# oceanusxiv/pathtracer-rs

Measured on AMD Instinct MI355X. Metric: Mray/s, Cornell Box 1024x1024, 256 spp, depth 15 (Msample/s in config), higher is better.
Workload: dtype f32

## Files before the change

pathtracer-rs_amd/csrc/ptrs_hip.hip:

```cpp
#include <hip/hip_runtime.h>

#include <cstdio>
#include <cstdlib>
#include <cstring>
#include <map>
#include <mutex>
#include <new>
#include <string>
#include <thread>
#include <vector>

#include "pt_render.h"
#include "pt_aov.h"
#include "pt_probe.h"

using namespace pt;

static const unsigned char k_sobol_blob[] = {
#include "sobol_tables_data.inc"
};

namespace {

thread_local std::string g_err;

struct Options {
    int lanes = 0;
    int refill = -1;
    int refill_connect = -1;
    int stack_lds = 8;
    int grid_mult = 0;
    int grid_pct = 0;
    int whole_rounds = 0;
    int persist = 1;
    int node_form = 0;
    int node_order = 0;
    int vote = -1;
    int fused_epilogue = 1;
    int fused_resolve = 1;
    int shade_lds = 1;
    int env_presample = 1;
    int peer_copy = 1;
    int deal = 0;
    int tail = 1;
    int tail_at = -1;
    int tail_paths = 0;
    int workspace_pct = 40;
    int aov_fused_film = 1;
};
Options g_opt;
std::mutex g_opt_mu;
Options options() { std::lock_guard<std::mutex> lk(g_opt_mu); return g_opt; }
struct OptionDesc { const char *name; int Options::*field; int lo, hi; };
const OptionDesc k_options[] = {
    {"lanes", &Options::lanes, 0, 8}, {"refill", &Options::refill, -1, 64}, {"refill_connect", &Options::refill_connect, -1, 64}, {"stack_lds", &Options::stack_lds, 8, 16},
    {"grid_mult", &Options::grid_mult, 0, 64}, {"persist", &Options::persist, 0, 1}, {"whole_rounds", &Options::whole_rounds, 0, 1}, {"grid_pct", &Options::grid_pct, 0, 100}, {"node_form", &Options::node_form, 0, 2}, {"node_order", &Options::node_order, 0, 1}, {"vote", &Options::vote, -1, 2}, {"shade_lds", &Options::shade_lds, 0, 1}, {"fused_epilogue", &Options::fused_epilogue, 0, 1}, {"fused_resolve", &Options::fused_resolve, 0, 1}, {"workspace_pct", &Options::workspace_pct, 1, 90}, {"peer_copy", &Options::peer_copy, 0, 1}, {"env_presample", &Options::env_presample, 0, 1}, {"deal", &Options::deal, 0, 1}, {"tail", &Options::tail, 0, 1}, {"tail_at", &Options::tail_at, -1, 64}, {"tail_paths", &Options::tail_paths, 0, 1 << 20}, {"aov_fused_film", &Options::aov_fused_film, 0, 1},
};

#define HIPCHK(expr)                                                                                             \
    do {                                                                                                          \
        hipError_t e_ = (expr);                                                                                   \
        if (e_ != hipSuccess) {                                                                                   \
            g_err = std::string(#expr) + ": " + hipGetErrorString(e_);                                            \
            return PTRS_ERR_DEVICE;                                                                               \
        }                                                                                                         \
    } while (0)

constexpr int BLOCK = 256, WAVES = BLOCK / 64;

__device__ inline uint32_t rfl(uint32_t v) { return (uint32_t)__builtin_amdgcn_readfirstlane((int)v); }
__device__ inline uint32_t lanes_below(unsigned long long m) { return __builtin_amdgcn_mbcnt_hi((uint32_t)(m >> 32), __builtin_amdgcn_mbcnt_lo((uint32_t)m, 0u)); }
__device__ inline uint32_t wave_push(uint32_t &count, bool pred) {
    const unsigned long long m = __ballot(pred);
    const uint32_t slot = count + lanes_below(m);
    count += (uint32_t)__popcll(m);
    return slot;
}
enum : uint32_t { TK_SUB = 64, TK_SUB_STRIDE = 32, TK_LAUNCH_WORDS = TK_SUB * TK_SUB_STRIDE };
__device__ inline uint32_t seg_next(uint32_t *ticket, uint32_t G) {
    const uint32_t per = (G + TK_SUB - 1u) / TK_SUB;
    const uint32_t home = (blockIdx.x * WAVES + (threadIdx.x >> 6)) & (TK_SUB - 1u);
    for (;;) {
        uint32_t tmp; unsigned long long open;
        asm volatile("v_mbcnt_lo_u32_b32 %0, -1, 0\n\tv_mbcnt_hi_u32_b32 %0, -1, %0\n\tv_lshlrev_b32 %0, 7, %0\n\tglobal_load_dword %0, %0, %2 sc1\n\ts_waitcnt vmcnt(0)\n\tv_cmp_gt_u32 %1, %3, %0"
                     : "=&v"(tmp), "=s"(open) : "s"(ticket), "s"(per) : "memory");
        static_assert(TK_SUB_STRIDE * 4u == 128u, "the asm above shifts the lane id by 7");
        if (open == 0ull) return 0xffffffffu;
        const unsigned long long rot = home ? ((open >> home) | (open << (64u - home))) : open;
        const uint32_t c = (home + (uint32_t)__ffsll((long long)rot) - 1u) & (TK_SUB - 1u);
        uint32_t t = 0;
        if (__lane_id() == 0) t = atomicAdd(ticket + c * TK_SUB_STRIDE, 1u);
        t = rfl(t);
        const uint32_t s = c * per + t;
        if (t < per && s < G) return s;
    }
}
__device__ inline uint32_t *seg_count(const DQueues &Q, uint32_t row, int q, uint32_t G, uint32_t s) { return Q.counts + ((size_t)row * Q_STRIDE + (size_t)q) * G + s; }
enum { TK_EXTEND = 0, TK_CONNECT = 1, TK_SHADE0 = 2, TK_EPILOGUE = 9, TK_RESOLVE = 10, TK_PRESAMPLE = 11, TK_TAIL = 12 };
__device__ inline bool round_is_dead(const DQueues &Q, uint32_t it) { return it > 0u && rfl(Q.alive[it]) == 0u; }

typedef __attribute__((address_space(3))) const v4 lds_v4;
__device__ inline v4 lds_ld(lds_v4 *q) { v4 r; r.x = q->x; r.y = q->y; r.z = q->z; r.w = q->w; return r; }
enum : uint32_t { TOP_LDS_STRIDE = 9 };
struct GeomTop {
    lds_v4 *top; const v4 *nodesv; const DTri *tris; uint32_t ktop;
    __device__ inline void node8(uint32_t i, v4 *o) const {
        if (i < ktop) { lds_v4 *q = top + TOP_LDS_STRIDE * i; for (int k = 0; k < 8; ++k) o[k] = lds_ld(q + k); }
        else { const v4 *q = nodesv + 8u * i; for (int k = 0; k < 8; ++k) o[k] = q[k]; }
    }
    __device__ inline void quad_load(uint32_t i, uint32_t px, uint32_t py, uint32_t pz, v4 &xn, v4 &xf, v4 &yn, v4 &yf, v4 &zn, v4 &zf, v4 &refs, v4 &meta) const {
        if (i < ktop) {
            typedef __attribute__((address_space(3))) const char lds_c;
            lds_c *b = (lds_c *)top + i * (TOP_LDS_STRIDE * 16u);
            xn = lds_ld((lds_v4 *)(b + px)); xf = lds_ld((lds_v4 *)(b + (px ^ 16u)));
            yn = lds_ld((lds_v4 *)(b + py)); yf = lds_ld((lds_v4 *)(b + (py ^ 16u)));
            zn = lds_ld((lds_v4 *)(b + pz)); zf = lds_ld((lds_v4 *)(b + (pz ^ 16u)));
            refs = lds_ld((lds_v4 *)(b + 96u)); meta = lds_ld((lds_v4 *)(b + 112u));
        } else {
            const char *b = reinterpret_cast<const char *>(nodesv);
            const uint32_t off = i * 128u;
            xn = *reinterpret_cast<const v4 *>(b + (size_t)(off + px)); xf = *reinterpret_cast<const v4 *>(b + (size_t)((off + px) ^ 16u));
            yn = *reinterpret_cast<const v4 *>(b + (size_t)(off + py)); yf = *reinterpret_cast<const v4 *>(b + (size_t)((off + py) ^ 16u));
            zn = *reinterpret_cast<const v4 *>(b + (size_t)(off + pz)); zf = *reinterpret_cast<const v4 *>(b + (size_t)((off + pz) ^ 16u));
            refs = *reinterpret_cast<const v4 *>(b + (size_t)(off + 96u)); meta = *reinterpret_cast<const v4 *>(b + (size_t)(off + 112u));
        }
    }
    __device__ inline void node(uint32_t, v4 &, v4 &, v4 &, v4 &) const {}
    __device__ inline void tri(uint32_t k, v4 &a, v4 &b, v4 &c) const { const v4 *q = reinterpret_cast<const v4 *>(tris + k); a = q[0]; b = q[1]; c = q[2]; }
};

struct StackSpill { unsigned long long *p; uint32_t stride; };
template <int D, bool OVF>
struct LdsStack {
    unsigned long long *col, *ovf; uint32_t ovf_stride;
    int n;
    __device__ inline void init(unsigned long long *lds, const StackSpill &sp) { col = lds + threadIdx.x; ovf = OVF ? sp.p + (size_t)blockIdx.x * BLOCK + threadIdx.x : nullptr; ovf_stride = sp.stride; n = 0; }
    __device__ inline void push(uint32_t v, float t) {
        const unsigned long long e = (unsigned long long)v | ((unsigned long long)f2u(t) << 32);
        if (!OVF || n < D) col[n * BLOCK] = e; else ovf[(size_t)(n - D) * ovf_stride] = e;
// ... 591 lines not shown
            __builtin_amdgcn_global_load_lds((gptr *)&pslot(P.pre0, m.e), (lptr *)(lds_pf + (5u * 4u + wv) * 64u), 16, 0, 0);
            __builtin_amdgcn_global_load_lds((gptr *)&pslot(P.pre1, m.e), (lptr *)(lds_pf + (6u * 4u + wv) * 64u), 16, 0, 0);
        }
    };
    const MatEntry *__restrict__ queue = Q.mat[MAT] + (size_t)s * seg_cap;
    const uint32_t n = rfl(*seg_count(Q, it, Q_MAT0 + MAT, Gn, s));
    if (n == 0) return;
    const uint32_t next_base = rfl(*seg_count(Q, it + 1u, Q_EXT, Gn, s)), nee_base = rfl(*seg_count(Q, it, Q_NEE, Gn, s));
    const uint32_t e_next0 = s * seg_cap + next_base, f0 = s * seg_cap + nee_base;
    uint32_t c_next = 0, c_nee = 0, c_shadow = 0, c_mis = 0;
    uint32_t i = lane;
    MatEntry m, m1; m.e = m.pid = m1.e = m1.pid = 0;
    if (i < n) { m = pslot(queue, i); dma(m); }
    if (i + 64u < n) m1 = pslot(queue, i + 64u);
    __builtin_amdgcn_s_waitcnt(0x0F70);
    while (i < n) {
        PathIn in;
        {
            lds_v4 *q = (lds_v4 *)lds_pf + threadIdx.x;
            if (FEAT & FEAT_IMAGE) in.ro = X.ld(q); else in.ro = mkv4(splat3(0.0f), 0.0f);
            in.rd = X.ld(q + BLOCK); in.beta = X.ld(q + 2 * BLOCK);
            const v4 a = X.ld(q + 3 * BLOCK), c = X.ld(q + 4 * BLOCK);
            in.st.x = f2u(a.x); in.st.y = f2u(a.y); in.st.z = f2u(a.z); in.st.w = f2u(a.w);
            in.hit.x = f2u(c.x); in.hit.y = f2u(c.y); in.hit.z = f2u(c.z); in.hit.w = f2u(c.w);
            if ((FEAT & FEAT_INFINITE) && cfg.pre_li != 0xffffffffu) { in.pre0 = X.ld(q + 5 * BLOCK); in.pre1 = X.ld(q + 6 * BLOCK); } else in.pre0 = in.pre1 = mkv4(splat3(0.0f), 0.0f);
        }
        __builtin_amdgcn_s_waitcnt(0xC07F);
        const uint32_t i2 = i + 64u;
        if (i2 < n) dma(m1);
        MatEntry m2; m2.e = m2.pid = 0;
        if (i2 + 64u < n) m2 = pslot(queue, i2 + 64u);
#ifdef PTRS_STAMPS
        const ShadeResult r = shade_item<MAT, FEAT>(R, S, C, sc, P, m.pid, in, X, stamp_acc, stamp_last);
#else
        const ShadeResult r = shade_item<MAT, FEAT>(R, S, C, sc, P, m.pid, in, X);
#endif
        err_dim = err_dim || r.err_dim;
        const uint32_t e_next = e_next0 + wave_push(c_next, r.next), f = f0 + wave_push(c_nee, r.nee);
        X.before_stores();
        store_shade_out(P, par ^ 1u, r, e_next, f);
        if (r.next) pslot(Q.ext[par ^ 1u], e_next) = m.pid;
        if (r.nee) pslot(Q.nee, f) = r.nee_entry(m.pid);
#ifdef PTRS_STAMPS
        { const unsigned long long t_ = __builtin_amdgcn_s_memtime(); stamp_acc[8] += t_ - stamp_last; stamp_last = t_; stamp_acc[10] += 1; }
#endif
        c_shadow += (uint32_t)__popcll(__ballot(r.shadow));
        c_mis += (uint32_t)__popcll(__ballot(r.mis));
        if (R.row_cost && (r.shadow || r.mis)) atomicAdd(R.row_cost + sample_row_of(R, m.pid), (r.shadow ? 1u : 0u) + (r.mis ? 1u : 0u));
        i = i2; m = m1; m1 = m2;
    }
    if (lane == 0) {
        *seg_count(Q, it + 1u, Q_EXT, Gn, s) = next_base + c_next;
        if (c_next) Q.alive[it + 1u] = 1u;
        *seg_count(Q, it, Q_NEE, Gn, s) = nee_base + c_nee;
        *seg_count(Q, it, Q_SHADOW, Gn, s) += c_shadow;
        *seg_count(Q, it, Q_MIS, Gn, s) += c_mis;
    }
}

template <int MAT, int FEAT, bool ENVPRE>
__global__ __launch_bounds__(BLOCK, (ShadeWaves<MAT, FEAT>::N)) void k_shade(DParams R, DSampler S, DCamera C, DScene sc, DPaths P, DQueues Q, uint32_t it, uint32_t seg_cap, ShadeLdsCfg cfg, uint32_t Gn, uint32_t *ticket) {
    __shared__ v4 lds_pf[ShadeLdsSizes<FEAT, ENVPRE>::NPF * BLOCK];
    __shared__ uint32_t lds_sob[SH_SOB_WORDS];
    __shared__ v4 lds_tri[SH_TRI_V4];
    __shared__ v4 lds_light[SH_LIGHTS * SH_LIGHT_V4];
    __shared__ float lds_marg[ShadeLdsSizes<FEAT, ENVPRE>::MARG ? SH_MARG_WORDS : 1];
    bool err_dim = false;
    if (round_is_dead(Q, it)) return;
    const ShadeCtxLds<ENVPRE> X = stage_shade_tables<FEAT, ENVPRE>(S, sc, cfg, lds_sob, lds_tri, lds_light, lds_marg);
    __syncthreads();
#ifdef PTRS_STAMPS
    unsigned long long stamp_acc[12] = {0, 0, 0, 0, 0, 0, 0, 0, 0, 0, 0, 0}, stamp_last = __builtin_amdgcn_s_memtime();
    for (uint32_t s = seg_next(ticket, Gn); s < Gn; s = seg_next(ticket, Gn)) shade_segment<MAT, FEAT, ENVPRE>(R, S, C, sc, P, Q, it, seg_cap, Gn, s, X, lds_pf, err_dim, stamp_acc, stamp_last);
#else
    for (uint32_t s = seg_next(ticket, Gn); s < Gn; s = seg_next(ticket, Gn)) shade_segment<MAT, FEAT, ENVPRE>(R, S, C, sc, P, Q, it, seg_cap, Gn, s, X, lds_pf, err_dim);
#endif
    if (err_dim) atomicOr(&Q.stats[CNT_ERR], (unsigned long long)PTRS_ERRFLAG_SOBOL_DIM);
#ifdef PTRS_STAMPS
    { const unsigned long long t_ = __builtin_amdgcn_s_memtime(); stamp_acc[11] += t_ - stamp_last; }
    if ((threadIdx.x & 63u) == 0) for (int k = 0; k < 12; ++k) atomicAdd(&Q.stats[CNT_STAMP0 + k], stamp_acc[k]);
#endif
}

template <int MAT, int FEAT, int GEOM, bool OVF, int DEPTH = 8>
__global__ __launch_bounds__(BLOCK, 2) void k_tail(DParams R, DSampler S, DCamera C, DScene sc, StackSpill spill, DPaths P, DQueues Q, uint32_t it0, uint32_t it_end, uint32_t seg_cap, uint32_t thresh_e, uint32_t thresh_c,
                                                   uint32_t kinds_mask, ShadeLdsCfg cfg, uint32_t Gn, uint32_t *ticket) {
    constexpr int FEAT_T = FEAT_SIMPLE;
    constexpr bool VOTE_C = GEOM == 0;
    __shared__ unsigned long long lds_stack[DEPTH * BLOCK];
    __shared__ v4 lds_geom[TravLds<DEPTH, GEOM>::V4];
    __shared__ v4 lds_pf[ShadeLdsSizes<FEAT, false>::NPF * BLOCK];
    __shared__ uint32_t lds_sob[4];
    __shared__ v4 lds_tri[SH_TRI_V4];
    __shared__ v4 lds_light[SH_LIGHTS * SH_LIGHT_V4];
    __shared__ float lds_marg[ShadeLdsSizes<FEAT, false>::MARG ? SH_MARG_WORDS : 1];
    if (round_is_dead(Q, it0)) return;
    LdsGeom LG; LG.root = LG.tri0 = LG.tri_copy = 0;
    const GeomTop GG = stage_top(sc, lds_geom, TravLds<DEPTH, GEOM>::TOP);
    if (GEOM > 0) LG = stage_lds_form(sc, lds_geom);
    cfg.sob_n = 0;
    const ShadeCtxLds<false> X = stage_shade_tables<FEAT, false>(S, sc, cfg, lds_sob, lds_tri, lds_light, lds_marg);
    __syncthreads();
    LdsStack<DEPTH, OVF> stk; stk.init(lds_stack, spill);
    uint32_t nn = 0, nt = 0; StepCount stepc;
    bool err_dim = false;
#ifdef PTRS_STAMPS
    unsigned long long stamp_acc[12] = {0, 0, 0, 0, 0, 0, 0, 0, 0, 0, 0, 0}, stamp_last = __builtin_amdgcn_s_memtime();
#endif
    for (uint32_t s = seg_next(ticket, Gn); s < Gn; s = seg_next(ticket, Gn)) {
        for (uint32_t it = it0; it < it_end; ++it) {
            if (rfl(*(volatile uint32_t *)seg_count(Q, it, Q_EXT, Gn, s)) == 0u) break;
#ifdef PTRS_STAMPS_EXT
            { unsigned long long xs[12] = {0, 0, 0, 0, 0, 0, 0, 0, 0, 0, 0, 0}, xs_last = 0; extend_segment<FEAT_T, DEPTH, OVF, GEOM, true>(R, sc, P, Q, it, seg_cap, thresh_e, kinds_mask, Gn, s, GG, LG, stk, nn, nt, stepc PT_XS_ARGS); }
#else
            extend_segment<FEAT_T, DEPTH, OVF, GEOM, true>(R, sc, P, Q, it, seg_cap, thresh_e, kinds_mask, Gn, s, GG, LG, stk, nn, nt, stepc);
#endif
            __threadfence_block();
#ifdef PTRS_STAMPS
            shade_segment<MAT, FEAT, false>(R, S, C, sc, P, Q, it, seg_cap, Gn, s, X, lds_pf, err_dim, stamp_acc, stamp_last);
#else
            shade_segment<MAT, FEAT, false>(R, S, C, sc, P, Q, it, seg_cap, Gn, s, X, lds_pf, err_dim);
#endif
            __threadfence_block();
            connect_segment<FEAT_T, DEPTH, OVF, GEOM, VOTE_C>(sc, P, Q, it, seg_cap, thresh_c, 1u, Gn, s, GG, LG, stk, nn, nt, stepc);
            __threadfence_block();
        }
    }
    if (err_dim) atomicOr(&Q.stats[CNT_ERR], (unsigned long long)PTRS_ERRFLAG_SOBOL_DIM);
    if (R.counters_on) { atomicAdd(&Q.stats[CNT_NODES], (unsigned long long)nn); atomicAdd(&Q.stats[CNT_TRIS], (unsigned long long)nt); atomicAdd(&Q.stats[CNT_NODE_STEPS], (unsigned long long)stepc.node_steps); atomicAdd(&Q.stats[CNT_NODE_VISITS], (unsigned long long)stepc.node_visits); atomicAdd(&Q.stats[CNT_TRI_STEPS], (unsigned long long)stepc.tri_steps); }
}

template <int FEAT>
__global__ __launch_bounds__(BLOCK) void k_env_presample(DSampler S, DScene sc, DPaths P, DQueues Q, uint32_t it, uint32_t seg_cap, uint32_t nee_kinds, uint32_t env_li, ShadeLdsCfg cfg, uint32_t Gn, uint32_t *ticket) {
    __shared__ float lds_marg[SH_MARG_WORDS];
    __shared__ uint32_t lds_sob[SH_SOB_WORDS];
    if (round_is_dead(Q, it)) return;
    const DLight &Le = sc.lights[env_li];
    {
        const uint32_t stride = sob_stride(cfg.sob_nib), nw = cfg.sob_nib * 16u;
        for (uint32_t i = threadIdx.x; i < cfg.sob_n * stride; i += BLOCK) { const uint32_t d = i / stride, w = i - d * stride; lds_sob[i] = w < nw ? S.nibtab[((size_t)(cfg.sob_lo + d) * SOBOL_NIBBLES) * 16u + w] : 0u; }
        const uint32_t nv = (uint32_t)Le.nv, gv = Le.guide_v;
        for (uint32_t i = threadIdx.x; i < nv; i += BLOCK) lds_marg[i] = sc.distdata[Le.fint_off + i];
        for (uint32_t i = threadIdx.x; i < nv + 1u; i += BLOCK) lds_marg[SH_MARG_N + i] = sc.distdata[Le.mcdf_off + i];
        for (uint32_t i = threadIdx.x; i < gv + 1u; i += BLOCK) lds_marg[2u * SH_MARG_N + 1u + i] = sc.distdata[Le.mguide_off + i];
    }
    __syncthreads();
    InfMarginal marg; marg.func = lds_marg; marg.cdf = lds_marg + SH_MARG_N; marg.guide = lds_marg + 2 * SH_MARG_N + 1;
    ShadeCtxLds<false> X; X.sob = (lds_u32 *)lds_sob; X.tris = nullptr; X.lights = nullptr; X.cfg = cfg; X.marg = marg;
    const uint32_t lane = __lane_id();
    for (uint32_t s = seg_next(ticket, Gn); s < Gn; s = seg_next(ticket, Gn)) {
        for (int m = 0; m < 6; ++m) {
            if (!(nee_kinds & (1u << m))) continue;
            const MatEntry *__restrict__ queue = Q.mat[m] + (size_t)s * seg_cap;
            const uint32_t n = rfl(*seg_count(Q, it, Q_MAT0 + m, Gn, s));
            for (uint32_t i = lane; i < n; i += 64u) {
                const MatEntry me = pslot(queue, i);
                const u4 stv = pslot(P.st, me.pid);
                const uint32_t field = f2u(pslot(P.ray_d[it & 1u], me.e).w) & ST_DIM_MASK;
                const VertexDims V = vertex_dims(field, true);
                const uint64_t index = (uint64_t)stv.x | ((uint64_t)stv.y << 32);
                const uint32_t dc[1] = {V.nee[4]};
                float uc[1];
                X.sobol<1>(S, index, dc, stv.w, uc);
                const float fl = floor_(uc[0] * (float)sc.n_lights);
                uint32_t li = fl > 0.0f ? (uint32_t)fl : 0u;
                if (li > sc.n_lights - 1u) li = sc.n_lights - 1u;
                if (li != env_li) continue;
                const uint32_t dn[2] = {V.nee[0], V.nee[1]};
                float u[2];
                X.sobol<2>(S, index, dn, stv.w, u);
                f3 wi, rgb; float pdf;
                const bool ok = inf_light_sample(sc, Le, mk2(u[0], u[1]), wi, pdf, rgb, &marg);
                pslot(P.pre0, me.e) = mkv4(wi, pdf);
                pslot(P.pre1, me.e) = mkv4(rgb, u2f(ok ? 1u : 0u));
            }
        }
    }
}

__global__ __launch_bounds__(BLOCK) void k_reduce_counts(const uint32_t *__restrict__ counts, uint32_t G, uint32_t *__restrict__ totals) {
    __shared__ uint32_t acc;
    if (threadIdx.x == 0) acc = 0;
    __syncthreads();
    uint32_t v = 0;
    for (uint32_t b = threadIdx.x; b < G; b += BLOCK) v += counts[(size_t)blockIdx.x * G + b];
    for (int off = 32; off > 0; off >>= 1) v += (uint32_t)__shfl_down((int)v, off);
    if ((threadIdx.x & 63) == 0) atomicAdd(&acc, v);
    __syncthreads();
    if (threadIdx.x == 0) totals[blockIdx.x] = acc;
}

__global__ __launch_bounds__(BLOCK) void k_film(DParams R, DSampler S, DPaths P, const float *__restrict__ table, v4 *film, int32_t y0, int32_t y1, int32_t tiles_x) {
// ... 546 lines not shown
        (void)hipMemsetAsync(Q.tickets, 0, ((size_t)rows * Q_STRIDE * TK_LAUNCH_WORDS + rows) * 4, stream);
    }
    void generate() { t0(T_AUX); hipLaunchKernelGGL(k_generate, dim3((G + WAVES - 1) / WAVES), dim3(BLOCK), 0, stream, R, S, C, P, Q, seg_cap, G, (uint32_t)deal_by_region()); t1(); }
    int deal_by_region() const { return opt.deal; }

    typedef void (*TravFn)(DParams, DScene, StackSpill, DPaths, DQueues, uint32_t, uint32_t, uint32_t, uint32_t, uint32_t, uint32_t *);
#define PTRS_PICK(K, D, O, GE) (v ? (TravFn)K<FEAT, D, O, GE, true> : (TravFn)K<FEAT, D, O, GE, false>)
#define PTRS_PICK_ALL(K) (ps->stack_lds == 9 ? PTRS_PICK(K, 9, false, 544) : ps->stack_lds == 8 ? (geom4 <= 640 ? (ovf ? PTRS_PICK(K, 8, true, 640) : PTRS_PICK(K, 8, false, 640)) : geom4 <= 1536 ? (ovf ? PTRS_PICK(K, 8, true, 1536) : PTRS_PICK(K, 8, false, 1536)) : (ovf ? PTRS_PICK(K, 8, true, 0) : PTRS_PICK(K, 8, false, 0))) \
                                              : (ovf ? PTRS_PICK(K, 16, true, 0) : PTRS_PICK(K, 16, false, 0)))
    template <int FEAT> TravFn pick_extend(bool v, bool ovf) { return PTRS_PICK_ALL(k_extend_rf); }
    template <int FEAT> TravFn pick_connect(bool v, bool ovf) { return PTRS_PICK_ALL(k_connect_rf); }
#undef PTRS_PICK_ALL
#undef PTRS_PICK
    StackSpill lane_spill() { StackSpill sp = ps->spill; if (sp.p) sp.p += (size_t)cur * ps->spill_lane_elems; return sp; }

    template <int FEAT> void extend_t(uint32_t it) {
        const StackSpill sp = lane_spill();
        const uint32_t epi_mask = opt.fused_epilogue ? kinds_mask : 0u;
        const TravFn fn = pick_extend<FEAT>(vote, sp.p != nullptr);
        hipLaunchKernelGGL(fn, dim3(persistent_grid(fn, T_EXTEND)), dim3(BLOCK), 0, stream, R, sc, sp, P, Q, it, seg_cap, refill, epi_mask, G, ticket(it, TK_EXTEND));
        if (epi_mask) return;
        t1(); t0(T_AUX);
        hipLaunchKernelGGL((k_epilogue<FEAT>), dim3(persistent_grid(k_epilogue<FEAT>, T_AUX)), dim3(BLOCK), 0, stream, R, sc, P, Q, it, kinds_mask, seg_cap, G, ticket(it, TK_EPILOGUE));
    }
    void extend(uint32_t it) { t0(T_EXTEND); if (feat_trace == FEAT_FULL) extend_t<FEAT_FULL>(it); else if (feat_trace == FEAT_IMG_ENV) extend_t<FEAT_IMG_ENV>(it); else extend_t<FEAT_SIMPLE>(it); t1(); }
    template <int FEAT> void connect_t(uint32_t it) {
        const StackSpill sp = lane_spill();
        const uint32_t fused = (opt.fused_epilogue && opt.fused_resolve) ? 1u : 0u;
        const TravFn fn = pick_connect<FEAT>(vote_connect, sp.p != nullptr);
        hipLaunchKernelGGL(fn, dim3(persistent_grid(fn, T_CONNECT)), dim3(BLOCK), 0, stream, R, sc, sp, P, Q, it, seg_cap, refill_connect, fused, G, ticket(it, TK_CONNECT));
        if (fused) return;
        t1(); t0(T_AUX);
        hipLaunchKernelGGL((k_resolve<FEAT>), dim3(persistent_grid(k_resolve<FEAT>, T_AUX)), dim3(BLOCK), 0, stream, sc, P, Q, it, seg_cap, G, ticket(it, TK_RESOLVE));
    }
    void connect(uint32_t it) { t0(T_CONNECT); if (feat_trace == FEAT_FULL) connect_t<FEAT_FULL>(it); else if (feat_trace == FEAT_IMG_ENV) connect_t<FEAT_IMG_ENV>(it); else connect_t<FEAT_SIMPLE>(it); t1(); }
    ShadeLdsCfg shade_cfg(uint32_t it) const {
        ShadeLdsCfg c;
        c.sob_nib = (2u * S.log2_res + (31u - (uint32_t)__builtin_clz(S.spp)) <= 32u) ? 8u : (uint32_t)SOBOL_NIBBLES;
        const uint32_t cap = SH_SOB_WORDS / sob_stride(c.sob_nib), top = std::min<uint32_t>(1024u, 3u + 8u * it + 9u);
        c.sob_lo = top > cap ? top - cap : 0u; c.sob_n = top - c.sob_lo;
        c.tri_lds = (sc.n_prims * SH_TRI_REC_V4 <= SH_TRI_V4 && opt.shade_lds) ? 1u : 0u;
        c.n_lights_lds = opt.shade_lds ? std::min<uint32_t>(sc.n_lights, SH_LIGHTS) : 0u;
        if (!opt.shade_lds) c.sob_n = 0;
        c.pre_li = presample_li();
        c.marg_li = 0xffffffffu;
        if (opt.shade_lds && !ps->H.inf_lights.empty()) {
            const DLight &Le = ps->H.lights[ps->H.inf_lights[0]];
            if (Le.nv >= 1 && (uint32_t)Le.nv <= SH_MARG_N && Le.guide_v >= 1 && Le.guide_v <= SH_MARG_N) c.marg_li = ps->H.inf_lights[0];
        }
        return c;
    }
    typedef void (*ShadeFn)(DParams, DSampler, DCamera, DScene, DPaths, DQueues, uint32_t, uint32_t, ShadeLdsCfg, uint32_t, uint32_t *);
    template <int FEAT, bool ENVPRE> ShadeFn shade_fn_t(int kind) {
        switch (kind) {
            case 0: return k_shade<0, FEAT, ENVPRE>;
            case 1: return k_shade<1, FEAT, ENVPRE>;
            case 2: return k_shade<2, FEAT, ENVPRE>;
            case 3: return k_shade<3, FEAT, ENVPRE>;
            case 4: return k_shade<4, FEAT, ENVPRE>;
            default: return k_shade<5, FEAT, ENVPRE>;
        }
    }
    bool env_presampled_only() const { return presample_li() != 0xffffffffu && ps->H.inf_lights.size() == 1; }
    ShadeFn shade_fn(int kind) {
        if (feat == FEAT_SIMPLE) return shade_fn_t<FEAT_SIMPLE, false>(kind);
        if (feat == FEAT_IMG) return shade_fn_t<FEAT_IMG, false>(kind);
        if (feat == FEAT_IMG_ENV) return env_presampled_only() ? shade_fn_t<FEAT_IMG_ENV, true>(kind) : shade_fn_t<FEAT_IMG_ENV, false>(kind);
        return env_presampled_only() ? shade_fn_t<FEAT_FULL, true>(kind) : shade_fn_t<FEAT_FULL, false>(kind);
    }
    uint32_t presample_li() const {
        if (!opt.env_presample || !(feat & FEAT_INFINITE) || S.kind != PTRS_SAMPLER_SOBOL || ps->H.inf_lights.empty()) return 0xffffffffu;
        const DLight &Le = ps->H.lights[ps->H.inf_lights[0]];
        return (Le.nv >= 1 && (uint32_t)Le.nv <= SH_MARG_N && Le.guide_v >= 1 && Le.guide_v <= SH_MARG_N) ? ps->H.inf_lights[0] : 0xffffffffu;
    }
    void presample(uint32_t it) {
        const uint32_t li = presample_li();
        const uint32_t nee_kinds = kinds_mask & 0x3fu & ~((1u << PTRS_MAT_MIRROR) | (1u << PTRS_MAT_GLASS));
        if (li == 0xffffffffu || !nee_kinds) return;
        t0(T_AUX);
        if (feat == FEAT_IMG_ENV) hipLaunchKernelGGL((k_env_presample<FEAT_IMG_ENV>), dim3(persistent_grid(k_env_presample<FEAT_IMG_ENV>, T_AUX)), dim3(BLOCK), 0, stream, S, sc, P, Q, it, seg_cap, nee_kinds, li, shade_cfg(it), G, ticket(it, TK_PRESAMPLE));
        else hipLaunchKernelGGL((k_env_presample<FEAT_FULL>), dim3(persistent_grid(k_env_presample<FEAT_FULL>, T_AUX)), dim3(BLOCK), 0, stream, S, sc, P, Q, it, seg_cap, nee_kinds, li, shade_cfg(it), G, ticket(it, TK_PRESAMPLE));
        t1();
    }
    typedef void (*TailFn)(DParams, DSampler, DCamera, DScene, StackSpill, DPaths, DQueues, uint32_t, uint32_t, uint32_t, uint32_t, uint32_t, uint32_t, ShadeLdsCfg, uint32_t, uint32_t *);
    enum : uint32_t { TAIL_PATHS_DEFAULT = 192 };
    TailFn tail_fn() {
        if (!opt.tail || !opt.fused_epilogue || !opt.fused_resolve || !opt.shade_lds || !opt.persist || (ps->stack_lds != 8 && ps->stack_lds != 9) || feat_trace != FEAT_SIMPLE || S.kind != PTRS_SAMPLER_SOBOL) return nullptr;
        int kind = -1;
        for (int k = 0; k < 7; ++k) if (ps->H.kinds_present[k]) { if (kind >= 0) return nullptr; kind = k; }
        const bool ovf = ps->spill.p != nullptr;
        if (ps->stack_lds == 9) return (kind == PTRS_MAT_MATTE && feat == FEAT_SIMPLE) ? (TailFn)k_tail<PTRS_MAT_MATTE, FEAT_SIMPLE, 544, false, 9> : nullptr;
        if (kind == PTRS_MAT_MATTE && feat == FEAT_SIMPLE) {
            if (geom4 <= 640) return ovf ? (TailFn)k_tail<PTRS_MAT_MATTE, FEAT_SIMPLE, 640, true> : (TailFn)k_tail<PTRS_MAT_MATTE, FEAT_SIMPLE, 640, false>;
            if (geom4 <= 1536) return ovf ? (TailFn)k_tail<PTRS_MAT_MATTE, FEAT_SIMPLE, 1536, true> : (TailFn)k_tail<PTRS_MAT_MATTE, FEAT_SIMPLE, 1536, false>;
            return ovf ? (TailFn)k_tail<PTRS_MAT_MATTE, FEAT_SIMPLE, 0, true> : (TailFn)k_tail<PTRS_MAT_MATTE, FEAT_SIMPLE, 0, false>;
        }
        if (kind == PTRS_MAT_DISNEY && feat == FEAT_IMG && geom4 > 1536) return ovf ? (TailFn)k_tail<PTRS_MAT_DISNEY, FEAT_IMG, 0, true> : (TailFn)k_tail<PTRS_MAT_DISNEY, FEAT_IMG, 0, false>;
        return nullptr;
    }
    uint32_t tail_round(uint32_t n_paths, uint32_t n_rounds) {
        if (!tail_fn()) return 0xffffffffu;
        if (opt.tail_at >= 0) return (uint32_t)opt.tail_at < n_rounds ? (uint32_t)opt.tail_at : 0xffffffffu;
        const double limit = (double)(opt.tail_paths > 0 ? (uint32_t)opt.tail_paths : (uint32_t)TAIL_PATHS_DEFAULT) * (double)G;
        const std::vector<double> &f = ps->alive_frac;
        for (uint32_t it = 0; it < n_rounds && it < f.size(); ++it) if (f[it] * (double)n_paths <= limit) return it;
        return 0xffffffffu;
    }
    uint32_t tail_at_last = 0xffffffffu;
    void tail(uint32_t it0, uint32_t it_end) {
        const TailFn fn = tail_fn();
        if (!fn) return;
        t0(T_TAIL);
        hipLaunchKernelGGL(fn, dim3(persistent_grid(fn, T_TAIL)), dim3(BLOCK), 0, stream, R, S, C, sc, lane_spill(), P, Q, it0, it_end, seg_cap, refill, refill_connect, kinds_mask & 0x3fu, shade_cfg(it0), G, ticket(it0, TK_TAIL));
        t1();
        tail_at_last = it0;
    }
    void learn(const uint32_t *counts, uint32_t n_rows, uint32_t n_paths) {
        if (!n_paths || n_paths < 4096u) return;
        std::vector<double> f(n_rows);
        for (uint32_t i = 0; i < n_rows; ++i) f[i] = (double)counts[(size_t)i * Q_STRIDE + Q_EXT] / (double)n_paths;
        ps->alive_frac.swap(f);
    }
    void shade(uint32_t it, int kind) {
        t0(T_SHADE);
        if (kind > 5) kind = 5;
        const ShadeFn fn = shade_fn(kind);
        hipLaunchKernelGGL(fn, dim3(persistent_grid(fn, T_SHADE)), dim3(BLOCK), 0, stream, R, S, C, sc, P, Q, it, seg_cap, shade_cfg(it), G, ticket(it, TK_SHADE0 + kind));
        t1();
    }
    void reduce_counts(uint32_t n_rows) { hipLaunchKernelGGL(k_reduce_counts, dim3(n_rows * Q_STRIDE), dim3(BLOCK), 0, stream, (const uint32_t *)Q.counts, G, (uint32_t *)ps->totals[cur].p); }
    uint32_t read_count(uint32_t it, int q) {
        std::vector<uint32_t> seg(G);
        (void)hipMemcpyAsync(seg.data(), Q.counts + ((size_t)it * Q_STRIDE + (size_t)q) * G, (size_t)G * 4, hipMemcpyDeviceToHost, stream);
        if (hipStreamSynchronize(stream) != hipSuccess) { rc = PTRS_ERR_DEVICE; return 0; }
        uint64_t t = 0; for (uint32_t v : seg) t += v;
        return t > 0xffffffffull ? 0xffffffffu : (uint32_t)t;
    }
    void read_counts(uint32_t *dst, uint32_t n_rows) {
        reduce_counts(n_rows);
        (void)hipMemcpyAsync(dst, ps->totals[cur].p, (size_t)n_rows * Q_STRIDE * 4, hipMemcpyDeviceToHost, stream);
        if (hipStreamSynchronize(stream) != hipSuccess) rc = PTRS_ERR_DEVICE;
    }
    void film(v4 *film_px, int32_t y0, int32_t y1) {
        const int32_t tiles_x = (R.W + 15) / 16, tiles_y = (y1 - y0 + 15) / 16;
        if (n_lanes > 1 && film_prev) (void)hipStreamWaitEvent(stream, film_prev, 0);
        t0(T_FILM); hipLaunchKernelGGL(k_film, dim3((uint32_t)tiles_x * (uint32_t)tiles_y), dim3(BLOCK), 0, stream, R, S, P, (const float *)ps->table.p, film_px, y0, y1, tiles_x); t1();
        if (n_lanes > 1) { film_prev = ps->lane_ev[cur]; (void)hipEventRecord(film_prev, stream); }
    }
    PtrsFilmPixel *host_film = nullptr; int32_t film_w = 0;
    void publish_rows(v4 *film_px, int32_t y0, int32_t y1) {
        if (!host_film || hipStreamSynchronize(stream) != hipSuccess) { rc = host_film ? PTRS_ERR_DEVICE : rc; return; }
        const size_t off = (size_t)y0 * (size_t)film_w, cnt = (size_t)(y1 - y0) * (size_t)film_w;
        if (hipMemcpyAsync(host_film + off, film_px + off, cnt * sizeof(PtrsFilmPixel), hipMemcpyDeviceToHost, stream) != hipSuccess || hipStreamSynchronize(stream) != hipSuccess) rc = PTRS_ERR_DEVICE;
    }
    void dump_rays(uint32_t it, const RayDump &d) {
        DevBuf cnt;
        if (cnt.ensure(16) != PTRS_OK) { rc = PTRS_ERR_DEVICE; return; }
        (void)hipMemsetAsync(cnt.p, 0, 16, stream);
        hipLaunchKernelGGL(k_dump_rays, dim3((G + WAVES - 1) / WAVES), dim3(BLOCK), 0, stream, P, Q, it, seg_cap, G, d.max_rays, d.out, (uint32_t *)cnt.p);
        uint32_t n = 0;
        if (hipMemcpyAsync(&n, cnt.p, 4, hipMemcpyDeviceToHost, stream) != hipSuccess || hipStreamSynchronize(stream) != hipSuccess) rc = PTRS_ERR_DEVICE;
        *d.n_out = n < d.max_rays ? n : d.max_rays;
        cnt.release();
    }
    bool aov_band = false;
    int aov_band_begin(uint64_t n, std::string &err) {
        for (auto &b : ps->aov_band) if ((rc = b.ensure((size_t)n * 16)) != PTRS_OK) { err = g_err + " (feature-plane band arrays)"; return rc; }
        if ((rc = ps->aov_band_pfilm.ensure((size_t)n * 8)) != PTRS_OK) { err = g_err + " (feature-plane band arrays)"; return rc; }
        aov_band = true;
        return PTRS_OK;
    }
    DAov aov_arrays(bool depth_plane) const {
        DAov A;
        if (aov_band) { A.albedo = (v4 *)ps->aov_band[0].p; A.normal = (v4 *)ps->aov_band[1].p; A.pos = (v4 *)ps->aov_band[2].p; A.depthp = depth_plane ? (v4 *)ps->aov_band[3].p : nullptr; A.pfilm = (f2a *)ps->aov_band_pfilm.p; }
        else { A.albedo = P.sh_o; A.normal = P.sh_d; A.pos = P.mis_o; A.depthp = depth_plane ? P.mis_d : nullptr; A.pfilm = nullptr; }
        return A;
    }
    bool aov_depth_plane(uint32_t planes) const { return !opt.aov_fused_film && (planes & PTRS_AOV_DEPTH) != 0; }
    void aov(uint32_t planes, uint32_t off) {
        t0(T_AUX);
        const DAov A = aov_arrays(aov_depth_plane(planes));
        if (feat == FEAT_SIMPLE) hipLaunchKernelGGL((k_aov<FEAT_SIMPLE>), dim3((G + WAVES - 1) / WAVES), dim3(BLOCK), 0, stream, R, C, sc, P, Q, A, off, seg_cap, G);
        else hipLaunchKernelGGL((k_aov<FEAT_FULL>), dim3((G + WAVES - 1) / WAVES), dim3(BLOCK), 0, stream, R, C, sc, P, Q, A, off, seg_cap, G);
        t1();
    }
    void film_aov(uint32_t planes, const DAovFilm &films, int32_t y0, int32_t y1, const DParams &Rf ) {
        const int32_t tiles_x = (R.W + 15) / 16, tiles_y = (y1 - y0 + 15) / 16;
        const DAov A = aov_arrays(aov_depth_plane(planes));
        DPaths Pf = P;
        if (A.pfilm) Pf.pfilm = A.pfilm;
        if (n_lanes > 1 && film_prev) (void)hipStreamWaitEvent(stream, film_prev, 0);
        if (opt.aov_fused_film) {
            DAovFilm F = films;
            for (uint32_t k = 0; k < AOV_PLANES; ++k) if (!(planes & (1u << k))) F.plane[k] = nullptr;
            t0(T_FILM); hipLaunchKernelGGL(k_film_aov, dim3((uint32_t)tiles_x * (uint32_t)tiles_y), dim3(BLOCK), 0, stream, Rf, S, Pf, A, (const float *)ps->table.p, F, y0, y1, tiles_x); t1();
        } else {
// ... 44 lines not shown
int do_render(PtrsScene *ps, const PtrsCamera *cam, const PtrsRenderParams *prm, v4 *film_dev, float *samples_dev, hipStream_t stream, PtrsStats *stats, const int32_t *single_pixel = nullptr,
              const RenderProgress *progress = nullptr, PtrsFilmPixel *host_film = nullptr, int share = 1, const RayDump *dump = nullptr, uint32_t *row_cost_dev = nullptr) {
    if (!ps || !cam || !prm || (!film_dev && !single_pixel && !row_cost_dev)) { g_err = "null argument"; return PTRS_ERR_INVALID; }
    HIPCHK(hipSetDevice(ps->device));
    HipBackend be;
    be.ps = ps; be.stream = stream; be.opt = scene_options(ps); be.host_film = host_film; be.film_w = prm->width; be.share = share;
    if (dump && be.opt.lanes == 0) be.opt.lanes = 1;
    int rc = get_sobol(ps->device, &be.sob);
    if (rc != PTRS_OK) return rc;
    std::string err;
    rc = render_impl(be, ps->sc, ps->H, ps->H.max_depth, *cam, *prm, film_dev, samples_dev, stats, err, progress, dump, single_pixel, row_cost_dev);
    if (rc != PTRS_OK) { if (!err.empty()) g_err = err; return rc; }
    if (be.rc != PTRS_OK) { if (g_err.empty()) g_err = "device error during render"; return be.rc; }
    return PTRS_OK;
}

int aov_check_args(PtrsScene *scene, const PtrsCamera *camera, const PtrsRenderParams *params, uint32_t planes, const void *const *plane_ptrs) {
    if (!scene || !camera || !params) { g_err = "null argument"; return PTRS_ERR_INVALID; }
    if (planes == 0u || (planes & ~(uint32_t)(PTRS_AOV_ALBEDO | PTRS_AOV_NORMAL | PTRS_AOV_DEPTH)) != 0u) { g_err = "planes must be a non-empty set of PTRS_AOV_* bits"; return PTRS_ERR_INVALID; }
    for (uint32_t k = 0; k < AOV_PLANES; ++k)
        if ((planes & (1u << k)) && (!plane_ptrs || !plane_ptrs[k])) { g_err = "null plane pointer for a requested plane"; return PTRS_ERR_INVALID; }
    int ndev = 0;
    if (hipGetDeviceCount(&ndev) != hipSuccess || ndev <= 0) { g_err = "no HIP device available (this library has no CPU fallback)"; return PTRS_ERR_DEVICE; }
    return PTRS_OK;
}

int do_render_aov(PtrsScene *ps, const PtrsCamera *cam, const PtrsRenderParams *prm, uint32_t planes, const DAovFilm &films, float *samples_dev, hipStream_t stream, PtrsStats *stats) {
    HIPCHK(hipSetDevice(ps->device));
    HipBackend be;
    be.ps = ps; be.stream = stream; be.opt = scene_options(ps); be.film_w = prm->width;
    int rc = get_sobol(ps->device, &be.sob);
    if (rc != PTRS_OK) return rc;
    std::string err;
    rc = render_aov_impl(be, ps->sc, ps->H, ps->H.max_depth, *cam, *prm, planes, films, samples_dev, stats, err);
    if (rc != PTRS_OK) { if (!err.empty()) g_err = err; return rc; }
    if (be.rc != PTRS_OK) { if (g_err.empty()) g_err = "device error during render"; return be.rc; }
    return PTRS_OK;
}

template <class F> int guarded(F &&f) {
    try { return f(); }
    catch (const std::bad_alloc &) { g_err = "out of host memory"; return PTRS_ERR_DEVICE; }
    catch (const std::exception &e) { g_err = std::string("internal error: ") + e.what(); return PTRS_ERR_INVALID; }
    catch (...) { g_err = "internal error"; return PTRS_ERR_INVALID; }
}

}

extern "C" {

int ptrs_abi_version(void) { return PTRS_ABI_VERSION; }
#ifndef PTRS_BUILD_ID
#define PTRS_BUILD_ID "unknown"
#endif
const char *ptrs_build_id(void) { return PTRS_BUILD_ID; }
const char *ptrs_last_error(void) { return g_err.c_str(); }

int ptrs_abi_sizeof(int which) {
    switch (which) {
        case 0: return (int)sizeof(PtrsTexture); case 1: return (int)sizeof(PtrsMaterial); case 2: return (int)sizeof(PtrsMesh);
        case 3: return (int)sizeof(PtrsLight); case 4: return (int)sizeof(PtrsBvhNode); case 5: return (int)sizeof(PtrsSceneDesc);
        case 6: return (int)sizeof(PtrsCamera); case 7: return (int)sizeof(PtrsRenderParams); case 8: return (int)sizeof(PtrsStats);
        case 9: return (int)sizeof(PtrsHit); case 10: return (int)sizeof(PtrsFilmPixel);
        default: return -1;
    }
}

int ptrs_set_option(const char *name, int64_t value) {
    if (!name) { g_err = "null option name"; return PTRS_ERR_INVALID; }
    for (const OptionDesc &o : k_options)
        if (!std::strcmp(name, o.name)) {
            if (value < o.lo || value > o.hi) { g_err = std::string("option ") + name + ": value outside [" + std::to_string(o.lo) + ", " + std::to_string(o.hi) + "]"; return PTRS_ERR_INVALID; }
            std::lock_guard<std::mutex> lk(g_opt_mu);
            g_opt.*(o.field) = (int)value;
            return PTRS_OK;
        }
    g_err = std::string("unknown option ") + name;
    return PTRS_ERR_INVALID;
}

int ptrs_get_option(const char *name, int64_t *value) {
    if (!name || !value) { g_err = "null argument"; return PTRS_ERR_INVALID; }
    for (const OptionDesc &o : k_options)
        if (!std::strcmp(name, o.name)) { std::lock_guard<std::mutex> lk(g_opt_mu); *value = g_opt.*(o.field); return PTRS_OK; }
    g_err = std::string("unknown option ") + name;
    return PTRS_ERR_INVALID;
}

static int scene_create_impl(const PtrsSceneDesc *desc, int32_t device, PtrsScene **out);
int ptrs_scene_create(const PtrsSceneDesc *desc, int32_t device, PtrsScene **out) { return guarded([&]() { return scene_create_impl(desc, device, out); }); }
static int scene_create_impl(const PtrsSceneDesc *desc, int32_t device, PtrsScene **out) {
    if (!desc || !out) { g_err = "null argument"; return PTRS_ERR_INVALID; }
    int ndev = 0;
    if (hipGetDeviceCount(&ndev) != hipSuccess || ndev <= 0) { g_err = "no HIP device available (this library has no CPU fallback)"; return PTRS_ERR_DEVICE; }
    if (device < 0 || device >= ndev) { g_err = "device ordinal out of range"; return PTRS_ERR_INVALID; }
    HIPCHK(hipSetDevice(device));
    PtrsScene *ps = new PtrsScene();
    ps->device = device;
    const Options opt = options();
    int rc = build_host_scene(*desc, ps->H, g_err, opt.node_form, opt.node_order);
    if (rc != PTRS_OK) { delete ps; return rc; }
    hipDeviceProp_t prop;
    if (hipGetDeviceProperties(&prop, device) == hipSuccess && prop.multiProcessorCount > 0) ps->n_cu = prop.multiProcessorCount;
    HostScene &H = ps->H;
    if ((rc = upload(ps->nodes2, H.nodes2)) || (rc = upload(ps->nodes4, H.nodes4)) || (rc = upload(ps->nodes, H.nodes)) || (rc = upload(ps->tris, H.tris)) || (rc = upload(ps->shade, H.shade)) || (rc = upload(ps->mats, H.mats)) ||
        (rc = upload(ps->texs, H.texs)) || (rc = upload(ps->levels, H.levels)) || (rc = upload(ps->texdata, H.texdata)) || (rc = upload(ps->lights, H.lights)) ||
        (rc = upload(ps->distdata, H.distdata)) || (rc = upload(ps->inf, H.inf_lights))) { delete ps; return rc; }
    DScene &sc = ps->sc;
    sc.nodes2 = (const DNode2 *)ps->nodes2.p; sc.n_nodes2 = (uint32_t)H.nodes2.size(); sc.nodes4 = (const DNode4 *)ps->nodes4.p; sc.n_nodes4 = (uint32_t)H.nodes4.size();
    sc.nodes = (const DNode *)ps->nodes.p; sc.tris = (const DTri *)ps->tris.p; sc.shade = (const DTriShade *)ps->shade.p; sc.mats = (const DMaterial *)ps->mats.p;
    sc.texs = (const DTexture *)ps->texs.p; sc.levels = (const DTexLevel *)ps->levels.p; sc.texdata = (const float *)ps->texdata.p; sc.lights = (const DLight *)ps->lights.p;
    sc.distdata = (const float *)ps->distdata.p; sc.inf_lights = (const uint32_t *)ps->inf.p;
    sc.n_nodes = (uint32_t)H.nodes.size(); sc.n_prims = (uint32_t)H.tris.size(); sc.n_lights = (uint32_t)H.lights.size(); sc.n_inf = (uint32_t)H.inf_lights.size();
    ps->stack_lds = (H.use_quad && opt.stack_lds == 16) ? 16u : 8u;
    if (!H.use_quad && opt.stack_lds != 16 && H.stack_bound == 9u && LN_V4 * (uint32_t)H.nodes2.size() + 9u * (uint32_t)H.tris.size() <= 544u) ps->stack_lds = 9u;
    if (H.stack_bound > ps->stack_lds) {
        const size_t threads = (size_t)ps->n_cu * 8 * BLOCK;
        ps->spill_lane_elems = threads * (size_t)(H.stack_bound - ps->stack_lds);
        if ((rc = ps->stack_spill.ensure(ps->spill_lane_elems * sizeof(unsigned long long))) != PTRS_OK) { delete ps; return rc; }
        ps->spill.p = (unsigned long long *)ps->stack_spill.p; ps->spill.stride = (uint32_t)threads;
    }
    *out = ps;
    return PTRS_OK;
}

void ptrs_scene_destroy(PtrsScene *scene) {
    if (!scene) return;
    (void)hipSetDevice(scene->device);
    delete scene;
}

int ptrs_scene_info(PtrsScene *scene, uint64_t *n_nodes, uint64_t *max_depth, uint64_t *n_tris) {
    if (!scene) { g_err = "null scene"; return PTRS_ERR_INVALID; }
    if (n_nodes) *n_nodes = scene->H.nodes.size();
    if (max_depth) *max_depth = scene->H.max_depth;
    if (n_tris) *n_tris = scene->H.tris.size();
    return PTRS_OK;
}

int ptrs_render_device(PtrsScene *scene, const PtrsCamera *camera, const PtrsRenderParams *params, void *film_inout_device, void *hip_stream, PtrsStats *stats) {
    return guarded([&]() { return do_render(scene, camera, params, (v4 *)film_inout_device, nullptr, (hipStream_t)hip_stream, stats); });
}

static int render_samples_impl(PtrsScene *scene, const PtrsCamera *camera, const PtrsRenderParams *params, PtrsFilmPixel *film_inout, float *sample_rgb, PtrsStats *stats);
int ptrs_render_samples(PtrsScene *scene, const PtrsCamera *camera, const PtrsRenderParams *params, PtrsFilmPixel *film_inout, float *sample_rgb, PtrsStats *stats) {
    return guarded([&]() { return render_samples_impl(scene, camera, params, film_inout, sample_rgb, stats); });
}
static int render_samples_impl(PtrsScene *scene, const PtrsCamera *camera, const PtrsRenderParams *params, PtrsFilmPixel *film_inout, float *sample_rgb, PtrsStats *stats) {
    if (!scene || !params || !film_inout) { g_err = "null argument"; return PTRS_ERR_INVALID; }
    HIPCHK(hipSetDevice(scene->device));
    const size_t npx = (size_t)params->width * (size_t)params->height;
    int rc = scene->film_tmp.ensure(npx * sizeof(PtrsFilmPixel));
    if (rc != PTRS_OK) return rc;
    int32_t rb = params->row_begin, re = params->row_end;
    if (re <= rb) { rb = 0; re = params->height; }
    if (rb < 0 || re > params->height) { g_err = "row band outside the film"; return PTRS_ERR_INVALID; }
    const size_t band_off = (size_t)rb * (size_t)params->width, band_px = (size_t)(re - rb) * (size_t)params->width;
    HIPCHK(hipMemcpy((PtrsFilmPixel *)scene->film_tmp.p + band_off, film_inout + band_off, band_px * sizeof(PtrsFilmPixel), hipMemcpyHostToDevice));
    float *sdev = nullptr; size_t sbytes = 0;
    if (sample_rgb) {
        const SampleGrid g = make_sample_grid(params->width, params->height, params->spp);
        const size_t spp = params->sampler == PTRS_SAMPLER_STRATIFIED ? (size_t)std::max(params->spp, 1) : (size_t)g.spp;
        sbytes = (size_t)g.NX * (size_t)g.NY * spp * 3 * sizeof(float);
        if ((rc = scene->samples_tmp.ensure(sbytes)) != PTRS_OK) return rc;
        HIPCHK(hipMemset(scene->samples_tmp.p, 0, sbytes));
        sdev = (float *)scene->samples_tmp.p;
    }
// ... 522 lines not shown
```

Before: 12570.

## Add grouped tail segments with wave-level queue merging and sized tail grid

After: 12580, median of 6. No clear change (+0.1%).

```diff
diff --git a/pathtracer-rs_amd/csrc/pt_tail_group.h b/pathtracer-rs_amd/csrc/pt_tail_group.h
--- /dev/null
+++ b/pathtracer-rs_amd/csrc/pt_tail_group.h
@@ -0,0 +1,33 @@
+#pragma once
+#include <stdint.h>
+
+#include "../../include/ptrs_detmath.h"
+
+namespace pt {
+
+enum : uint32_t { TAIL_GROUP_MAX = 64 };
+
+PT_HD uint32_t tail_group_tickets(uint32_t G, uint32_t k) { return (G + k - 1u) / k; }
+
+struct TailGroup { uint32_t s0, s1; };
+PT_HD TailGroup tail_group_of(uint32_t g, uint32_t k, uint32_t G) {
+    TailGroup t; t.s0 = g * k; t.s1 = t.s0 + k < G ? t.s0 + k : G;
+    return t;
+}
+
+PT_HD uint32_t tail_group_push(uint32_t off, uint32_t n, uint32_t seg_cap) {
+    if (off == 0xffffffffu || n > seg_cap || off + n > seg_cap) return 0xffffffffu;
+    return off + n;
+}
+PT_HD bool tail_group_merges(uint32_t total) { return total != 0xffffffffu; }
+
+PT_HD uint32_t tail_group_src(uint32_t s, uint32_t seg_cap, uint32_t i) { return s * seg_cap + i; }
+PT_HD uint32_t tail_group_dst(const TailGroup &t, uint32_t seg_cap, uint32_t off, uint32_t i) { return t.s0 * seg_cap + off + i; }
+
+PT_HD uint32_t tail_group_plan(const TailGroup &t, const uint32_t *counts, uint32_t seg_cap, uint32_t *off) {
+    uint32_t run = 0;
+    for (uint32_t j = 0; j < t.s1 - t.s0; ++j) { off[j] = run; run = tail_group_push(run, counts[j], seg_cap); }
+    return run;
+}
+
+}
diff --git a/pathtracer-rs_amd/csrc/ptrs_hip.hip b/pathtracer-rs_amd/csrc/ptrs_hip.hip
--- a/pathtracer-rs_amd/csrc/ptrs_hip.hip
+++ b/pathtracer-rs_amd/csrc/ptrs_hip.hip
@@ -13,6 +13,7 @@
 #include "pt_render.h"
 #include "pt_aov.h"
 #include "pt_probe.h"
+#include "pt_tail_group.h"
 
 using namespace pt;
 
@@ -45,16 +46,18 @@
     int tail = 1;
     int tail_at = -1;
     int tail_paths = 0;
+    int tail_group = 0;
     int workspace_pct = 40;
     int aov_fused_film = 1;
 };
+enum : int { TAIL_GROUP_DEFAULT = 1 };
 Options g_opt;
 std::mutex g_opt_mu;
 Options options() { std::lock_guard<std::mutex> lk(g_opt_mu); return g_opt; }
 struct OptionDesc { const char *name; int Options::*field; int lo, hi; };
 const OptionDesc k_options[] = {
     {"lanes", &Options::lanes, 0, 8}, {"refill", &Options::refill, -1, 64}, {"refill_connect", &Options::refill_connect, -1, 64}, {"stack_lds", &Options::stack_lds, 8, 16},
-    {"grid_mult", &Options::grid_mult, 0, 64}, {"persist", &Options::persist, 0, 1}, {"whole_rounds", &Options::whole_rounds, 0, 1}, {"grid_pct", &Options::grid_pct, 0, 100}, {"node_form", &Options::node_form, 0, 2}, {"node_order", &Options::node_order, 0, 1}, {"vote", &Options::vote, -1, 2}, {"shade_lds", &Options::shade_lds, 0, 1}, {"fused_epilogue", &Options::fused_epilogue, 0, 1}, {"fused_resolve", &Options::fused_resolve, 0, 1}, {"workspace_pct", &Options::workspace_pct, 1, 90}, {"peer_copy", &Options::peer_copy, 0, 1}, {"env_presample", &Options::env_presample, 0, 1}, {"deal", &Options::deal, 0, 1}, {"tail", &Options::tail, 0, 1}, {"tail_at", &Options::tail_at, -1, 64}, {"tail_paths", &Options::tail_paths, 0, 1 << 20}, {"aov_fused_film", &Options::aov_fused_film, 0, 1},
+    {"grid_mult", &Options::grid_mult, 0, 64}, {"persist", &Options::persist, 0, 1}, {"whole_rounds", &Options::whole_rounds, 0, 1}, {"grid_pct", &Options::grid_pct, 0, 100}, {"node_form", &Options::node_form, 0, 2}, {"node_order", &Options::node_order, 0, 1}, {"vote", &Options::vote, -1, 2}, {"shade_lds", &Options::shade_lds, 0, 1}, {"fused_epilogue", &Options::fused_epilogue, 0, 1}, {"fused_resolve", &Options::fused_resolve, 0, 1}, {"workspace_pct", &Options::workspace_pct, 1, 90}, {"peer_copy", &Options::peer_copy, 0, 1}, {"env_presample", &Options::env_presample, 0, 1}, {"deal", &Options::deal, 0, 1}, {"tail", &Options::tail, 0, 1}, {"tail_at", &Options::tail_at, -1, 64}, {"tail_paths", &Options::tail_paths, 0, 1 << 20}, {"tail_group", &Options::tail_group, 0, (int)TAIL_GROUP_MAX}, {"aov_fused_film", &Options::aov_fused_film, 0, 1},
 };
 
 #define HIPCHK(expr)                                                                                             \
@@ -812,9 +815,37 @@
 #endif
 }
 
+__device__ inline bool tail_merge_wave(const DPaths &P, const DQueues &Q, uint32_t it0, uint32_t seg_cap, uint32_t Gn, const TailGroup &tg) {
+    const uint32_t lane = __lane_id(), m = tg.s1 - tg.s0, par = it0 & 1u;
+    uint32_t *cnt = seg_count(Q, it0, Q_EXT, Gn, tg.s0);
+    const uint32_t n_mine = lane < m ? cnt[lane] : 0u;
+    uint32_t total = 0;
+    for (uint32_t j = 0; j < m; ++j) total = tail_group_push(total, (uint32_t)__builtin_amdgcn_readlane((int)n_mine, (int)j), seg_cap);
+    if (!tail_group_merges(total)) return false;
+    uint32_t off = rfl(n_mine);
+    if (total == off) return true;
+    uint32_t *const ext = Q.ext[par];
+    v4 *const ray_o = P.ray_o[par], *const ray_d = P.ray_d[par], *const beta = P.beta[par];
+    auto ld4 = [](const v4 *base, uint32_t i) { const v4 &q = pslot(base, i); v4 r; r.x = q.x; r.y = q.y; r.z = q.z; r.w = q.w; return r; };
+    for (uint32_t j = 1; j < m; ++j) {
+        const uint32_t n = (uint32_t)__builtin_amdgcn_readlane((int)n_mine, (int)j);
+        for (uint32_t i = lane; i < n; i += 64u) {
+            const uint32_t src = tail_group_src(tg.s0 + j, seg_cap, i), dst = tail_group_dst(tg, seg_cap, off, i);
+            const uint32_t pid = pslot(ext, src);
+            const v4 o = ld4(ray_o, src), d = ld4(ray_d, src), b = ld4(beta, src);
+            pslot(ext, dst) = pid;
+            pstore(ray_o, dst, o); pstore(ray_d, dst, d); pstore(beta, dst, b);
+        }
+        off = tail_group_push(off, n, seg_cap);
+    }
+    if (lane < m) cnt[lane] = lane == 0u ? total : 0u;
+    __threadfence_block();
+    return true;
+}
+
 template <int MAT, int FEAT, int GEOM, bool OVF, int DEPTH = 8>
 __global__ __launch_bounds__(BLOCK, 2) void k_tail(DParams R, DSampler S, DCamera C, DScene sc, StackSpill spill, DPaths P, DQueues Q, uint32_t it0, uint32_t it_end, uint32_t seg_cap, uint32_t thresh_e, uint32_t thresh_c,
-                                                   uint32_t kinds_mask, ShadeLdsCfg cfg, uint32_t Gn, uint32_t *ticket) {
+                                                   uint32_t kinds_mask, ShadeLdsCfg cfg, uint32_t Gn, uint32_t tail_group, uint32_t *ticket) {
     constexpr int FEAT_T = FEAT_SIMPLE;
     constexpr bool VOTE_C = GEOM == 0;
     __shared__ unsigned long long lds_stack[DEPTH * BLOCK];
@@ -837,7 +868,11 @@
 #ifdef PTRS_STAMPS
     unsigned long long stamp_acc[12] = {0, 0, 0, 0, 0, 0, 0, 0, 0, 0, 0, 0}, stamp_last = __builtin_amdgcn_s_memtime();
 #endif
-    for (uint32_t s = seg_next(ticket, Gn); s < Gn; s = seg_next(ticket, Gn)) {
+    const uint32_t Tn = tail_group_tickets(Gn, tail_group);
+    for (uint32_t g = seg_next(ticket, Tn); g < Tn; g = seg_next(ticket, Tn)) {
+        const TailGroup tg = tail_group_of(g, tail_group, Gn);
+        const uint32_t s_end = (tail_group > 1u && tail_merge_wave(P, Q, it0, seg_cap, Gn, tg)) ? tg.s0 + 1u : tg.s1;
+        for (uint32_t s = tg.s0; s < s_end; ++s)
         for (uint32_t it = it0; it < it_end; ++it) {
             if (rfl(*(volatile uint32_t *)seg_count(Q, it, Q_EXT, Gn, s)) == 0u) break;
 #ifdef PTRS_STAMPS_EXT
@@ -1550,10 +1585,13 @@
         else hipLaunchKernelGGL((k_env_presample<FEAT_FULL>), dim3(persistent_grid(k_env_presample<FEAT_FULL>, T_AUX)), dim3(BLOCK), 0, stream, S, sc, P, Q, it, seg_cap, nee_kinds, li, shade_cfg(it), G, ticket(it, TK_PRESAMPLE));
         t1();
     }
-    typedef void (*TailFn)(DParams, DSampler, DCamera, DScene, StackSpill, DPaths, DQueues, uint32_t, uint32_t, uint32_t, uint32_t, uint32_t, uint32_t, ShadeLdsCfg, uint32_t, uint32_t *);
+    typedef void (*TailFn)(DParams, DSampler, DCamera, DScene, StackSpill, DPaths, DQueues, uint32_t, uint32_t, uint32_t, uint32_t, uint32_t, uint32_t, ShadeLdsCfg, uint32_t, uint32_t, uint32_t *);
+    uint32_t tail_group() const { return opt.tail_group > 0 ? (uint32_t)opt.tail_group : (uint32_t)TAIL_GROUP_DEFAULT; }
     enum : uint32_t { TAIL_PATHS_DEFAULT = 192 };
     TailFn tail_fn() {
         if (!opt.tail || !opt.fused_epilogue || !opt.fused_resolve || !opt.shade_lds || !opt.persist || (ps->stack_lds != 8 && ps->stack_lds != 9) || feat_trace != FEAT_SIMPLE || S.kind != PTRS_SAMPLER_SOBOL) return nullptr;
+        const bool quad_geom = ps->stack_lds != 9 && geom4 > 1536;
+        if (opt.vote >= 0 && (opt.vote == 0 || (opt.vote == 1) != quad_geom)) return nullptr;
         int kind = -1;
         for (int k = 0; k < 7; ++k) if (ps->H.kinds_present[k]) { if (kind >= 0) return nullptr; kind = k; }
         const bool ovf = ps->spill.p != nullptr;
@@ -1569,7 +1607,7 @@
     uint32_t tail_round(uint32_t n_paths, uint32_t n_rounds) {
         if (!tail_fn()) return 0xffffffffu;
         if (opt.tail_at >= 0) return (uint32_t)opt.tail_at < n_rounds ? (uint32_t)opt.tail_at : 0xffffffffu;
-        const double limit = (double)(opt.tail_paths > 0 ? (uint32_t)opt.tail_paths : (uint32_t)TAIL_PATHS_DEFAULT) * (double)G;
+        const double limit = (double)(opt.tail_paths > 0 ? (uint32_t)opt.tail_paths : (uint32_t)TAIL_PATHS_DEFAULT) * (double)tail_group_tickets(G, tail_group());
         const std::vector<double> &f = ps->alive_frac;
         for (uint32_t it = 0; it < n_rounds && it < f.size(); ++it) if (f[it] * (double)n_paths <= limit) return it;
         return 0xffffffffu;
@@ -1579,7 +1617,9 @@
         const TailFn fn = tail_fn();
         if (!fn) return;
         t0(T_TAIL);
-        hipLaunchKernelGGL(fn, dim3(persistent_grid(fn, T_TAIL)), dim3(BLOCK), 0, stream, R, S, C, sc, lane_spill(), P, Q, it0, it_end, seg_cap, refill, refill_connect, kinds_mask & 0x3fu, shade_cfg(it0), G, ticket(it0, TK_TAIL));
+        const uint32_t k = tail_group(), need = (tail_group_tickets(G, k) + WAVES - 1) / WAVES, fit = resident_grid(fn);
+        last_grid[T_TAIL] = need < fit ? need : fit; last_per_cu[T_TAIL] = (uint32_t)wgs_per_cu(fn);
+        hipLaunchKernelGGL(fn, dim3(last_grid[T_TAIL]), dim3(BLOCK), 0, stream, R, S, C, sc, lane_spill(), P, Q, it0, it_end, seg_cap, refill, refill_connect, kinds_mask & 0x3fu, shade_cfg(it0), G, k, ticket(it0, TK_TAIL));
         t1();
         tail_at_last = it0;
     }
@@ -1790,7 +1830,12 @@
 int ptrs_get_option(const char *name, int64_t *value) {
     if (!name || !value) { g_err = "null argument"; return PTRS_ERR_INVALID; }
     for (const OptionDesc &o : k_options)
-        if (!std::strcmp(name, o.name)) { std::lock_guard<std::mutex> lk(g_opt_mu); *value = g_opt.*(o.field); return PTRS_OK; }
+        if (!std::strcmp(name, o.name)) {
+            std::lock_guard<std::mutex> lk(g_opt_mu);
+            *value = g_opt.*(o.field);
+            if (o.field == &Options::tail_group && *value == 0) *value = TAIL_GROUP_DEFAULT;
+            return PTRS_OK;
+        }
     g_err = std::string("unknown option ") + name;
     return PTRS_ERR_INVALID;
 }
```
